# submission2019/cnn-quantization

Measured on AMD Instinct MI355X. Metric: activation elements/sec (and % HBM peak) for per-channel int4 Q/DQ, ResNet-50 b512, higher is better.
Workload: dtype f32

## Files before the change

### cnn_quantization_amd/_lib.py

```python
import ctypes
import os

from . import _build

_P = ctypes.c_void_p
_I = ctypes.c_int
_L = ctypes.c_int64
_F = ctypes.c_float

STAT_MIN, STAT_MAX, STAT_MEAN, STAT_STD, STAT_B, STAT_KURT, STAT_STD_POS, NSTAT = 0, 1, 2, 3, 4, 5, 6, 7
MOM_MIN, MOM_MAX, MOM_SUM, MOM_SUMSQ, MOM_COUNT, MOM_SUM_RELU, MOM_SUMSQ_RELU, NMOM = 0, 1, 2, 3, 4, 5, 6, 7
DEV_ABS, DEV_Z4, NDEV = 0, 1, 2
QP_SCALE, QP_ZP, QP_QMAX, NQP = 0, 1, 2, 3
MT_DELTA, MT_CMIN, MT_CMAX, MT_OMEGA, MT_ALPHA, MT_WSTART, NMT = 0, 1, 2, 3, 4, 5, 6
MT_HIST_BINS = 131072
MT_HIST_WINDOW, MT_HIST_REPLICAS = 128, 256


def mt_hist_words(C):
    return MT_HIST_BINS + 2 + 2 * C + MT_HIST_REPLICAS * MT_HIST_WINDOW + 1
KLD_BINS, KLD_QBINS, KLD_NCAND = 2001, 15, 994
DIAG_BITS, DIAG_ALPHA, DIAG_DELTA, DIAG_OFFSET, NDIAG = 0, 1, 2, 3, 4
DTYPE_F32, DTYPE_BF16, DTYPE_F16, NDTYPE = 0, 1, 2, 3

# ... 29 lines not shown
    'cnnq_pc_qdq': (_I, [_P, _P, _L, _L, _L, _P, _P, _P, _I, _P]),
    'cnnq_pc_quantize_pack4': (_I, [_P, _P, _L, _L, _L, _P, _P]),
    'cnnq_pc_dequantize_pack4': (_I, [_P, _P, _L, _L, _L, _P, _P]),
    'cnnq_pc_quantize_u8': (_I, [_P, _P, _L, _L, _L, _P, _P]),
    'cnnq_pc_dequantize_u8': (_I, [_P, _P, _L, _L, _L, _P, _P]),
    'cnnq_pc_packed_layout': (_I, [_P, _L, _L, _P, _P]),
    'cnnq_pc_quantize_packed': (_I, [_P, _P, _L, _L, _L, _P, _P, _P, _P]),
    'cnnq_pc_quantize_packed_form': (_I, [_P, _P, _L, _L, _L, _P, _P, _P, _I, _P]),
    'cnnq_pc_dequantize_packed': (_I, [_P, _P, _L, _L, _L, _P, _P, _P, _P]),
    'cnnq_pc_dequantize_packed_form': (_I, [_P, _P, _L, _L, _L, _P, _P, _P, _I, _P]),
    'cnnq_xrank_window_bytes': (ctypes.c_size_t, [_I, _I]),
    'cnnq_xrank_alloc': (_I, [_I, _I, _P, _P]),
    'cnnq_pc_minmax_qdq_xrank': (_I, [_P, _P, _L, _L, _L, _I, _I, _P, _P, ctypes.c_size_t, _P, _I, _I, _I, ctypes.c_uint32, _P, _L,
                                      _P]),
    'cnnq_pc_minmax_qdq_xrank_dev': (_I, [_P, _P, _L, _L, _L, _I, _I, _P, _P, ctypes.c_size_t, _P, _I, _I, _I, _P, _P, _L, _P, _P, _P]),
    'cnnq_pc_minmax_qdq_xrank_seq': (_I, [_P, _P, _L, _L, _L, _I, _I, _P, _P, ctypes.c_size_t, _P, _I, _I, _I, ctypes.c_uint32, _P, _I, _P, _L,
                                          _P, _P, _P]),
    'cnnq_hist_replicas_fold': (_I, [_P, _P, _P]),
    'cnnq_pc_minmax': (_I, [_P, _L, _L, _L, _P, _P]),
    'cnnq_pc_minmax_strided': (_I, [_P, _L, _L, _L, _L, _P, _P]),
    'cnnq_pc_qdq_strided': (_I, [_P, _P, _L, _L, _L, _L, _P, _P, _P, _I, _P]),
    'cnnq_pc_minmax_reduce': (_I, [_P, _I, _L, _P, _P]),
    'cnnq_pc_minmax_params': (_I, [_P, _I, _L, _I, _I, _P, _P]),
    'cnnq_pc_minmax_qdq': (_I, [_P, _P, _L, _L, _L, _I, _I, _P, _P, _P, _P, _P]),
    'cnnq_pc_resident_describe': (_I, [_L, _L, _L, ctypes.POINTER(ctypes.c_int32)]),
    'cnnq_pc_minmax_qdq_resident': (_I, [_P, _P, _L, _L, _L, _I, _I, _P, _P, _P]),
    'cnnq_group_ws_alloc': (_I, [ctypes.c_size_t, ctypes.POINTER(ctypes.c_void_p)]),
    'cnnq_group_ws_free': (_I, [_P]),
    'cnnq_group_ws_status': (_I, [_P, ctypes.POINTER(ctypes.c_uint32)]),
    'cnnq_group_ws_status_clear': (_I, [_P]),
    'cnnq_pc_group_workspace': (ctypes.c_size_t, [_L, _L, _L]),
    'cnnq_group_ws_at_rest': (_I, [_P, ctypes.POINTER(ctypes.c_uint64)]),
    'cnnq_pc_group_describe': (_I, [_L, _L, _L, ctypes.POINTER(ctypes.c_int32)]),
    'cnnq_pc_minmax_qdq_group': (_I, [_P, _P, _L, _L, _L, _I, _I, _P, _P, _P, ctypes.c_uint32, _P]),
    'cnnq_pc_minmax_local': (_I, [_P, _L, _L, _L, _P, _P, _P]),
    'cnnq_pc_minmax_local_auto': (_I, [_P, _L, _L, _L, _P, _P, ctypes.c_size_t, _P, _P]),
    'cnnq_pc_gathered_qdq': (_I, [_P, _P, _L, _L, _L, _P, _I, _I, _I, _P, _P]),
    'cnnq_pc_minmax_qdq_workspace': (ctypes.c_size_t, [_L, _L, _L]),
    'cnnq_pc_minmax_qdq_auto': (_I, [_P, _P, _L, _L, _L, _I, _I, _P, _P, ctypes.c_size_t, _I, _P]),
    'cnnq_hist_replica_bytes': (ctypes.c_size_t, []),
    'cnnq_pc_minmax_qdq_single': (_I, [_P, _P, _L, _L, _L, _I, _I, _P, ctypes.c_size_t, _P, _P, _P, _P, _P, _P]),
    'cnnq_entropy_replicas': (_I, [_P, _P, _P]),
    'cnnq_entropy_replicas_batch': (_I, [_P, _I, _P, _P]),
    'cnnq_midtread_entropy_batch': (_I, [_I, _P, _P, _P, _P, _P, _P]),
    'cnnq_pc_aciq_workspace': (ctypes.c_size_t, [_L, _L, _L, _I]),
    'cnnq_pc_aciq_qdq': (_I, [_P, _P, _L, _L, _L, ctypes.POINTER(ParamsCfg), _P, _P, _P, _P]),
    'cnnq_pc_aciq_qdq_single': (_I, [_P, _P, _L, _L, _L, ctypes.POINTER(ParamsCfg), _P, _P, ctypes.c_size_t, _P, _P, _P, _P, _P,
                                     ctypes.c_uint32, _P]),
    'cnnq_pc_aciq_qdq_auto': (_I, [_P, _P, _L, _L, _L, ctypes.POINTER(ParamsCfg), _P, _P, ctypes.c_size_t, _P, _P, _P]),
    'cnnq_pc_aciq_fused_xrank': (_I, [_P, _P, _L, _L, _L, ctypes.POINTER(ParamsCfg), _P, _P, ctypes.c_size_t, _P, _P, _P, _P,
                                      ctypes.POINTER(XRankCtx), ctypes.c_uint32, _P]),
    'cnnq_pc_midtread_fused_xrank': (_I, [_P, _P, _L, _L, _L, ctypes.c_double, _I, _P, _I, _P, _P, ctypes.c_size_t, _P, _P, _P, _P,
                                          ctypes.POINTER(XRankCtx), ctypes.c_uint32, _P]),
    'cnnq_pc_stats_xrank': (_I, [_P, _L, _L, _L, _I, _I, _I, _P, _P, ctypes.c_size_t, _P, _P, ctypes.POINTER(XRankCtx), ctypes.c_uint32,
                                 _P]),
    'cnnq_pc_weight_correct': (_I, [_P, _L, _L, _P, _P, _I, _I, _P]),
    'cnnq_pc_bcorr_sums': (_I, [_P, _P, _L, _L, _L, _I, _P, _P]),
    'cnnq_pc_qdq_bcorr_sums': (_I, [_P, _L, _L, _L, _P, _I, _P, _P]),
    'cnnq_pc_qdq_bcorr': (_I, [_P, _P, _L, _L, _L, _P, _P, _I, _P]),
    'cnnq_pc_bcorr_bias': (_I, [_P, _I, _L, _P, _P, _P]),
    'cnnq_pc_bcorr_apply': (_I, [_P, _L, _L, _L, _P, _P]),
    'cnnq_pc_midtread_params': (_I, [_P, _L, ctypes.c_double, _I, _I, _P, _I, _P, _P]),
    'cnnq_pc_midtread_qdq': (_I, [_P, _P, _L, _L, _L, _P, _I, _P, _P, _P]),
    'cnnq_pc_midtread_qdq_single': (_I, [_P, _P, _L, _L, _L, ctypes.c_double, _I, _P, _I, _P, _P, ctypes.c_size_t, _P, _P, _P,
                                         ctypes.c_uint32, _P]),
    'cnnq_midtread_entropy': (_I, [_P, _P, _L, _L, _P, _P]),
# ... 93 lines not shown
```

### cnn_quantization_amd/csrc/cnnq_group.hip.h

```cpp
#pragma once
#include "cnnq_common.hip.h"
#include "cnnq_qdq.hip.h"
#include "cnnq_xrank.hip.h"
#include "cnnq_resident.hip.h"

namespace {

constexpr long long GRP_TIMEOUT_TICKS = 2000000;
constexpr long long GRP_TIMEOUT_SHORT = 50000;
constexpr int GRP_TIMEOUT_SPINS = 1 << 20;
constexpr int GRP_CNT_STRIDE = 64;
constexpr int GRP_GS_MAX = 512;
constexpr int GRP_GS_BIG = 704;
#ifndef GRP_ACQUIRE
#define GRP_ACQUIRE 0
#endif
constexpr int GRP_SUB = 16;
#ifndef GRP_K32_WAVES
#define GRP_K32_WAVES 3
#endif

#ifdef GRP_TRACE
__device__ unsigned long long* g_grp_trace = nullptr;
#define GRP_STAMP(i)                                                                                     \
// ... 311 lines not shown
                expired = (now - t0 > timeout_ticks || spins > GRP_TIMEOUT_SPINS) ? 1 : 0;
            }
            if (__builtin_amdgcn_readfirstlane(expired)) {
                if ((tid & 63) == 0) atomicOr(sh_code, 1);
                return;
            }
            if (spins < 2) __builtin_amdgcn_s_sleep(8);
            else if (spins < 6) __builtin_amdgcn_s_sleep(32);
            else __builtin_amdgcn_s_sleep(64);
        }
    }
    if (!whole_wg) {
        for (int m = L >> 1; m >= 1; m >>= 1) { tn = pmin(tn, shfl_xor_f(tn, m)); tx = pmax(tx, shfl_xor_f(tx, m)); }
        if (active && j == 0) { sh_mn[ch] = tn; sh_mx[ch] = tx; }
    }
}

struct GWs {
    unsigned* status;
    unsigned* cnt;
    unsigned long long* part;
    unsigned long long* slots;
    int gstride;
};

#ifndef FLAT_ABL
#define FLAT_ABL 0
#endif
#if FLAT_ABL & 1
#define FLAT_ABL_NOSTORE(o) && (o)[0] == 3.0e38f
#else
#define FLAT_ABL_NOSTORE(o)
#endif
template <int A, int K, int OUT = 0, bool XR = false>
__global__ void __launch_bounds__(TPB, (K == 32 ? GRP_K32_WAVES : 1)) k_mmq_group(
    const float* __restrict__ x, float* __restrict__ y, const Geo g, const int Gs, const int num_bits, const int positive,
    const GWs ws, float* __restrict__ qp, float* __restrict__ mm, const unsigned flags, const XOut xo = XOut{},
    const XRank xr = XRank{}) {
    if constexpr (XR) xr_prologue(xr);
    __shared__ float l_mn[TPB * A], l_mx[TPB * A];
    extern __shared__ unsigned cnnq_dyn_lds[];
    unsigned* const sh_hist = cnnq_dyn_lds;
    if constexpr (OUT == 1) {
        if (xo.hist) xhist_zero(sh_hist, 1 << (num_bits < 8 ? num_bits : 8));
    }
    __shared__ float sh_mn[MAXCH], sh_mx[MAXCH], sh_sc[MAXCH], sh_zp[MAXCH], sh_rs[MAXCH];
    __shared__ int sh_timed_out, sh_slow;
    if (threadIdx.x == 0) sh_slow = 0;
    const unsigned st0 = threadIdx.x == 0 ? __hip_atomic_load(ws.status, __ATOMIC_RELAXED, __HIP_MEMORY_SCOPE_AGENT) : 0u;
    GRP_STAMP(0);
    const RBlk rb = rblk_of(g, Gs);
    const Blk& b = rb.b;
    const int tid = threadIdx.x;
    const int col = b.col0 + tid;
    const bool ok = col < b.col1;
    const int colc = ok ? col : b.col0;
    const int nrows = b.n1 - b.n0;
    const size_t base = (size_t)b.n0 * (size_t)g.P + (size_t)colc * 4;

    float v[K][4];
#pragma unroll
    for (int j = 0; j < K; ++j) {
        const int r = j < nrows ? j : nrows - 1;
        ldv_nt<4>(x + base + (size_t)r * (size_t)g.P, v[j]);
    }
    __builtin_amdgcn_sched_barrier(0);
    GRP_STAMP(1);
    float mn[A], mx[A];
    bool nan = false;
#pragma unroll
    for (int a = 0; a < A; ++a) { mn[a] = INFINITY; mx[a] = -INFINITY; }
#pragma unroll
    for (int j = 0; j < K; ++j) lane_acc<A>(v[j], mn, mx, nan);
    if (A == 1 && nan) { mn[0] = NAN; mx[0] = NAN; }
    wg_channel_minmax<A>(g, b, ok, mn, mx, l_mn, l_mx, sh_mn, sh_mx);
    const int nch = b.c1 - b.c0;
    GRP_STAMP(2);

    unsigned long long* blk = ws.part + (size_t)rb.group * ws.gstride;
    const int kk = (g.mode == 1) ? 1 : g.k;
    const bool use_slots = (flags & MMQ_FLAG_SLOTS) != 0;
    unsigned long long* slots = ws.slots + (size_t)rb.group * ws.gstride;
    if (use_slots) {
        for (int ch = tid; ch < nch; ch += TPB)
            __hip_atomic_store(slots + (size_t)rb.member * kk + ch, slot_of(sh_mn[ch], sh_mx[ch]), __ATOMIC_RELAXED,
                               __HIP_MEMORY_SCOPE_AGENT);
        if (tid == 0) sh_timed_out = ((flags & MMQ_FLAG_TEST_HOOK) ? 2 : 0) | ((st0 & 1u) ? 4 : 0);
        __syncthreads();
        GRP_STAMP(3);
    } else {
    for (int ch = tid; ch < nch; ch += TPB)
        __hip_atomic_store(blk + (size_t)rb.member * kk + ch, pack_pair(sh_mn[ch], sh_mx[ch]), __ATOMIC_RELAXED,
                           __HIP_MEMORY_SCOPE_AGENT);
    asm volatile("s_waitcnt vmcnt(0)" ::: "memory");
    __syncthreads();
    GRP_STAMP(3);
    }
    float sn = INFINITY, sx = -INFINITY;
#if FLAT_ABL & 2
    if (tid == 0) sh_timed_out = 0;
    __syncthreads();
    if (true) {
    } else
#else
    if (use_slots) {
        const int c0 = sh_timed_out;
// ... 75 lines not shown
#pragma unroll
    for (int a = 0; a < A; ++a) {
        const unsigned e = (unsigned)colc * 4u + (unsigned)a;
        const int ch = (int)(e / (unsigned)g.HW) - b.c0;
        sc[a] = sh_sc[ch];
        zp[a] = sh_zp[ch];
    }

    unsigned nzp[A];
#pragma unroll
    for (int a = 0; a < A; ++a) nzp[a] = 0u;
    if (!__builtin_amdgcn_readfirstlane(sh_slow)) {
        float rs[A];
#pragma unroll
        for (int a = 0; a < A; ++a) {
            const unsigned e = (unsigned)colc * 4u + (unsigned)a;
            rs[a] = sh_rs[(int)(e / (unsigned)g.HW) - b.c0];
        }
#pragma unroll
        for (int j = 0; j < K; ++j) {
            if (j < nrows) {
                float o[4], cd[4];
                if constexpr (A == 1) {
                    qdq4_fast(v[j], sc[0], rs[0], zp[0], qm, o, cd);
                } else {
#pragma unroll
                    for (int e = 0; e < 4; ++e) o[e] = qdq1_fast(v[j][e], sc[e], rs[e], zp[e], qm, cd[e]);
                }
                if (ok FLAT_ABL_NOSTORE(o))
                    xstore<OUT, A>(xo, reinterpret_cast<char*>(y), xo.codes, xo.packed, (base + (size_t)j * (size_t)g.P) * 4, o,
                                   cd, sh_hist, zp, nzp);
            }
        }
    } else {
#pragma unroll
        for (int j = 0; j < K; ++j) {
            if (j < nrows) {
                float o[4], cd[4];
#pragma unroll
                for (int e = 0; e < 4; ++e) o[e] = qdq1(v[j][e], sc[A == 1 ? 0 : e], zp[A == 1 ? 0 : e], qm, cd[e]);
                if (ok FLAT_ABL_NOSTORE(o))
                    xstore<OUT, A>(xo, reinterpret_cast<char*>(y), xo.codes, xo.packed, (base + (size_t)j * (size_t)g.P) * 4, o,
                                   cd, sh_hist, zp, nzp);
            }
        }
    }
    if constexpr (OUT == 1) {
        if (xo.hist) xhist_flush<A>(sh_hist, xo.hist, 1 << (num_bits < 8 ? num_bits : 8), zp, nzp);
    }
    GRP_STAMP(6);
#if !(FLAT_ABL & 2)
    if (use_slots) {
        if (tid == 0) sh_timed_out = grp_depart_last(grp_lines(ws.cnt, rb.group, Gs, 0, 1), rb.member, Gs) ? 1 : 0;
        __syncthreads();
        if (sh_timed_out)
            for (int m = tid; m < Gs * kk; m += TPB) __hip_atomic_store(slots + m, 0ull, __ATOMIC_RELAXED, __HIP_MEMORY_SCOPE_AGENT);
    } else if (tid == 0) grp_depart(grp_lines(ws.cnt, rb.group, Gs, 0, 1), rb.member, Gs);
#endif
#ifdef GRP_TRACE
    if (g_grp_trace) {
        asm volatile("s_waitcnt vmcnt(0)" ::: "memory");
        __syncthreads();
        if (tid == 0) {
            g_grp_trace[(size_t)blockIdx.x * 16 + 8] = wall_clock64();
            g_grp_trace[(size_t)blockIdx.x * 16 + 7] = ((unsigned long long)__builtin_amdgcn_s_getreg((31 << 11) | 20) << 32) |
                                                       (unsigned)__builtin_amdgcn_s_getreg((31 << 11) | 4);
        }
    }
#endif
}

struct FGeo {
    int N, C, HW, P;
    unsigned cpc;
    unsigned total;
    int Gs;
// ... 414 lines not shown
```

### cnn_quantization_amd/csrc/cnnq_kernels.hip

```cpp

#include <string.h>

#include <vector>
#include "cnnq_common.hip.h"
#include "cnnq_stats.hip.h"
#include "cnnq_params.hip.h"
#include "cnnq_qdq.hip.h"
#include "cnnq_pack4.hip.h"
#include "cnnq_midtread.hip.h"
#include "cnnq_corrections.hip.h"
#include "cnnq_pertensor.hip.h"
#include "cnnq_resident.hip.h"
#include "cnnq_group.hip.h"
#include "cnnq_plan.hip.h"
#include "cnnq_kld.hip.h"
#include "cnnq_half.hip.h"
#include "cnnq_half_stats.hip.h"
#include "cnnq_half_bcorr.hip.h"
#include "cnnq_nhwc.hip.h"
#include "cnnq_nhwc_aciq.hip.h"
#include "cnnq_nhwc_collect.hip.h"
#include "cnnq_nhwc_bcorr.hip.h"
#include "cnnq_nhwc_midtread.hip.h"
#include "cnnq_nhwc_entropy.hip.h"
// ... 563 lines not shown
int cnnq_group_ws_status(const void* ws, uint32_t* status_host) {
    if (!ws || !status_host) return CNNQ_EINVAL;
    return (int)hipMemcpy(status_host, ws, sizeof(uint32_t), hipMemcpyDeviceToHost);
}

int cnnq_group_ws_status_clear(void* ws) {
    if (!ws) return CNNQ_EINVAL;
    const uint32_t zero = 0;
    return (int)hipMemcpy(ws, &zero, sizeof(uint32_t), hipMemcpyHostToDevice);
}

int cnnq_group_ws_at_rest(const void* ws, uint64_t* nonzero_words_host) {
    if (!ws || !nonzero_words_host) return CNNQ_EINVAL;
    std::vector<uint32_t> h(GRP_WS_PAIRS / 4);
    const hipError_t e = hipMemcpy(h.data(), ws, GRP_WS_PAIRS, hipMemcpyDeviceToHost);
    if (e != hipSuccess) return (int)e;
    constexpr size_t ptf0 = PTF_OFF / 4, ptf1 = (PTF_OFF + 256 + (size_t)PTF_MAX_ROWS * 16) / 4;
    uint64_t n = 0;
    for (size_t i = 1; i < h.size(); ++i) n += (i < ptf0 || i >= ptf1) && h[i] != 0u;
    *nonzero_words_host = n;
    return 0;
}

#ifdef GRP_TRACE
int cnnq_debug_group_trace(void* buf) {
    unsigned long long* p = reinterpret_cast<unsigned long long*>(buf);
    return (int)hipMemcpyToSymbol(HIP_SYMBOL(g_grp_trace), &p, sizeof(p));
}
#endif

int cnnq_pc_group_describe(int64_t N, int64_t C, int64_t HW, int32_t out[8]) {
    if (!out) return CNNQ_EINVAL;
    GPlan p;
    const int rc = plan_group(N, C, HW, true, &p, true, 1);
    if (rc) return rc;
    const int32_t vals[8] = {p.v.A, p.K + p.KL, p.g.mode, p.g.S, p.g.ncb, p.Gs, p.ngroups, p.g.S * p.g.ncb};
    for (int i = 0; i < 8; ++i) out[i] = vals[i];
    return 0;
}

int cnnq_pc_minmax_qdq_group(const float* x, float* y, int64_t N, int64_t C, int64_t HW, int num_bits, int positive,
                             void* ws, float* qp, float* mm, unsigned flags, void* stream) {
    if (!x || !y || !ws || !qp || num_bits < 1 || num_bits > 32 || misaligned(ws, 128)) return CNNQ_EINVAL;
    GPlan p;
    const int rc = plan_group(N, C, HW, al16(x) && al16(y), &p, true, flat_lds_rows(0, false));
    if (rc) return rc;
    return launch_group(x, y, p, num_bits, positive ? 1 : 0, ws, qp, mm, flags, (hipStream_t)stream);
}

int cnnq_pc_minmax_local(const float* x, int64_t N, int64_t C, int64_t HW, float* pmm, float* local, void* stream) {
    if (!x || !pmm || !local) return CNNQ_EINVAL;
    const int G = cnnq_pc_groups(N, C, HW, al16(x) ? 1 : 0);
    if (G <= 0) return g_error(G);
    const int rc = cnnq_pc_minmax(x, N, C, HW, pmm, stream);
    if (rc) return rc;
    return cnnq_pc_minmax_reduce(pmm, G, C, local, stream);
}

int cnnq_pc_minmax_local_auto(const float* x, int64_t N, int64_t C, int64_t HW, float* pmm, void* gws, size_t gws_bytes,
                              float* local, void* stream) {
    if (!x || !local) return CNNQ_EINVAL;
    static const int64_t max_bytes = env_int("CNNQ_LOCAL_GROUP_MAX_MB", 384) * ((int64_t)1 << 20);
    if (gws && !misaligned(gws, 128) && N * C * HW * 4 <= max_bytes) {
        GPlan p;
        if (plan_group(N, C, HW, al16(x), &p, false) == 0 && p.ws_bytes <= gws_bytes)
            return launch_minmax_group(x, p, gws, local, (hipStream_t)stream);
    }
    return cnnq_pc_minmax_local(x, N, C, HW, pmm, local, stream);
}

int cnnq_pc_gathered_qdq(const float* x, float* y, int64_t N, int64_t C, int64_t HW, const float* gathered, int W,
                         int num_bits, int positive, float* qp, void* stream) {
    if (!x || !y || !gathered || W <= 0 || num_bits < 1 || num_bits > 32) return CNNQ_EINVAL;
    Variant v;
    Geo g;
    const int rc = plan(N, C, HW, al16(x) && al16(y), 1, &v, &g, 1);
    if (rc) return rc;
    const GathArgs ga{W, num_bits, positive ? 1 : 0, qp};
// ... 20 lines not shown
}

int cnnq_pc_minmax_qdq_auto(const float* x, float* y, int64_t N, int64_t C, int64_t HW, int num_bits, int positive,
                            float* ws, void* gws, size_t gws_bytes, int allow_single_launch, void* stream) {
    if (!x || !y || !ws || num_bits < 1 || num_bits > 32 || C <= 0) return CNNQ_EINVAL;
    const MmWs w(ws, C);
    if (allow_single_launch) {
        const size_t gneed = gws ? cnnq_pc_group_workspace(N, C, HW) : 0;
        WPlan wp;
        int route = mm_route(N, C, HW, al16(x) && al16(y), gneed > 0 && gneed <= gws_bytes, &wp);
        if (route == ROUTE_GROUP) {
            const int rc = cnnq_pc_minmax_qdq_group(x, y, N, C, HW, num_bits, positive, gws, w.qp, w.mm, 0u, stream);
            if (rc != CNNQ_ENOTSUP) return rc;
            route = mm_route(N, C, HW, al16(x) && al16(y), false, &wp);
        }
        if (route == ROUTE_WHOLE) return launch_whole(x, y, wp, num_bits, positive ? 1 : 0, w.qp, w.mm, hs(stream));
    }
    return cnnq_pc_minmax_qdq(x, y, N, C, HW, num_bits, positive, w.pmm, w.qp, nullptr, nullptr, stream);
}

size_t cnnq_hist_replica_bytes(void) { return (size_t)XHIST_REPLICAS * 256 * sizeof(unsigned long long); }

int cnnq_pc_minmax_qdq_single(const float* x, float* y, int64_t N, int64_t C, int64_t HW, int num_bits, int positive,
                              void* gws, size_t gws_bytes, float* qp, float* mm, uint8_t* codes, uint64_t* hist_rep,
                              uint8_t* packed, void* stream) {
    if (!x || !qp || num_bits < 1 || num_bits > 32 || C <= 0) return CNNQ_EINVAL;
    if (packed ? (y || codes || hist_rep || num_bits > 4 || misaligned(packed, 2)) : !y) return CNNQ_EINVAL;
    if ((codes || hist_rep) && num_bits > 8) return CNNQ_EINVAL;
    if (misaligned(codes, 4) || misaligned(hist_rep, 8) || misaligned(gws, 128)) return CNNQ_EINVAL;
    const int out = packed ? 2 : (codes || hist_rep) ? 1 : 0;
    const XOut xo = xout(codes, hist_rep, packed);
    const bool al = al16(x) && (packed ? true : al16(y));
    GPlan gp;
    const bool group_ok = gws && plan_group(N, C, HW, al, &gp, true, flat_lds_rows(out, false)) == 0 && gp.ws_bytes <= gws_bytes;
    WPlan wp;
    switch (mm_route(N, C, HW, al, group_ok, &wp)) {
    case ROUTE_WHOLE: return launch_whole(x, y, wp, num_bits, positive ? 1 : 0, qp, mm, hs(stream), out, xo);
    case ROUTE_GROUP: return launch_group(x, y, gp, num_bits, positive ? 1 : 0, gws, qp, mm, 0u, hs(stream), out, xo);
    }
    return CNNQ_ENOTSUP;
}

size_t cnnq_xrank_window_bytes(int world, int cmax) {
    return (world > 0 && cmax > 0) ? xr_window_bytes(world, cmax) : 0;
}

int cnnq_xrank_alloc(int world, int cmax, void** window, unsigned char handle[64]) {
    if (!window || !handle || world <= 0 || cmax <= 0) return CNNQ_EINVAL;
    const size_t bytes = xr_window_bytes(world, cmax);
    hipError_t e = hipExtMallocWithFlags(window, bytes, hipDeviceMallocUncached);
    if (e != hipSuccess) return (int)e;
    e = hipMemset(*window, 0, bytes);
    hipIpcMemHandle_t h;
    if (e == hipSuccess) e = hipIpcGetMemHandle(&h, *window);
    if (e == hipSuccess) e = hipDeviceSynchronize();
    if (e != hipSuccess) {
        (void)hipFree(*window);
        *window = nullptr;
        return (int)e;
    }
    memcpy(handle, &h, 64);
    return 0;
}

static int xrank_launch(const float* x, float* y, int64_t N, int64_t C, int64_t HW, int num_bits, int positive, float* ws, void* gws,
                        size_t gws_bytes, void* const* windows, int rank, int world, int cmax, uint32_t seq, uint32_t* seq_dev,
                        uint32_t* status, int64_t timeout_ticks, uint8_t* codes, uint64_t* hist_rep, void* stream, int zero_c = 0,
// ... 1377 lines not shown
```

### cnn_quantization_amd/csrc/cnnq_plan.hip.h

```cpp
#pragma once
#include <stdio.h>
#include "cnnq_common.hip.h"
#include "cnnq_resident.hip.h"
#include "cnnq_group.hip.h"
#include "cnnq_aciq.hip.h"
#include "cnnq_stats1.hip.h"

namespace {

int gcd_i(int a, int b) { return b ? gcd_i(b, a % b) : a; }

constexpr int MAXG = 64;

int choose_variant(int64_t N, int64_t C, int64_t HW, bool aligned16, Variant* v) {
    if (aligned16 && HW % 4 == 0) {
        const int64_t cpc = HW / 4;
        int J = 4;
        if (cpc <= TPB * 4) {
            const int64_t smax = N < MAXG ? N : MAXG;
            for (J = 4; J > 1; J >>= 1) {
                const int64_t cap = TPB * J;
                const int64_t ncb = (cpc > cap) ? C * ((cpc + cap - 1) / cap) : (C + cap / cpc - 1) / (cap / cpc);
                static const int64_t minwgs = env_int("CNNQ_PLAN_MINWGS", 2048);
                if (ncb * smax >= minwgs) break;
// ... 278 lines not shown
    int64_t Gs = (total + TPB * (K + KL) - 1) / (TPB * (K + KL));
    int64_t gs_max = grp_gs_max();
    if (Gs > gs_max && K == 32 && lds_rows >= 1) {
        KL = 8;
        Gs = (total + TPB * (K + KL) - 1) / (TPB * (K + KL));
        gs_max = grp_gs_big();
    }
    if (Gs > gs_max || Gs < 2) return CNNQ_ENOTSUP;
    const int64_t rows = (TPB * (K + KL)) / cpc + 3;
    if (rows * C * HW * 4 >= (int64_t)1 << 32) return CNNQ_ENOTSUP;
    const int64_t nsub = (Gs + GRP_SUB - 1) / GRP_SUB;
    if (C * (nsub > 1 ? nsub + 1 : 1) > GRP_MAX_LINES) return CNNQ_ENOTSUP;
    p->flat = 1;
    p->KL = KL;
    p->v = {4, 1, 1};
    p->K = K;
    p->Gs = (int)Gs;
    p->ngroups = (int)C;
    p->gstride = (int)(((Gs + 15) / 16) * 16);
    p->ws_bytes = GRP_WS_PAIRS + (size_t)C * p->gstride * 8;
    FGeo& f = p->fg;
    f.N = (int)N; f.C = (int)C; f.HW = (int)HW; f.P = (int)(C * HW);
    f.cpc = (unsigned)cpc; f.total = (unsigned)total; f.Gs = (int)Gs;
    f.q256 = (unsigned)(TPB / cpc); f.r16 = (unsigned)(TPB % cpc) * 16u; f.rs = (unsigned)(C * HW * 4);
    static const int cb_knob = env_int("CNNQ_GRP_CB", 4);
    const int64_t cb_fit = ((int64_t)chip_cus() * 3 / 2) / Gs;
    f.cb = (int)(cb_knob > 1 ? (cb_fit < cb_knob ? (cb_fit < 1 ? 1 : cb_fit) : cb_knob) : 1);
    p->g = Geo{};
    p->g.N = (int)N; p->g.C = (int)C; p->g.HW = (int)HW; p->g.P = (int)(C * HW);
    p->g.mode = 3; p->g.S = (int)Gs; p->g.ncb = (int)C; p->g.Cn = (int)C; p->g.nb = 1; p->g.k = 1;
    return 0;
}

int plan_group_compute(int64_t N, int64_t C, int64_t HW, bool aligned16, GPlan* p, bool allow_flat, int lds_rows, int a4_kmax);

inline int flat_lds_rows(int out, bool xrank) {
    static const int kl_knob = env_int("CNNQ_FLAT_KL", 0);
    return (out == 1 || xrank) ? 0 : (kl_knob == 8 ? 2 : 1);
}

int plan_group(int64_t N, int64_t C, int64_t HW, bool aligned16, GPlan* p, bool allow_flat = true, int lds_rows = 0, int a4_kmax = 32) {
    struct Entry { int64_t N, C, HW; int key, rc; GPlan plan; };
    constexpr int SLOTS = 64;
    thread_local Entry cache[SLOTS];
    thread_local int used = 0, next = 0;
    const int key = (aligned16 ? 1 : 0) | (allow_flat ? 2 : 0) | (lds_rows << 2) | (a4_kmax << 4);
    for (int i = 0; i < used; ++i)
        if (cache[i].N == N && cache[i].C == C && cache[i].HW == HW && cache[i].key == key) {
            *p = cache[i].plan;
            return cache[i].rc;
        }
    const int rc = plan_group_compute(N, C, HW, aligned16, p, allow_flat, lds_rows, a4_kmax);
    Entry& e = cache[next];
    e.N = N; e.C = C; e.HW = HW; e.key = key; e.rc = rc; e.plan = *p;
    next = (next + 1) % SLOTS;
    if (used < SLOTS) ++used;
    return rc;
}

int plan_rows(int64_t N, int64_t C, int64_t HW, GPlan* p, int a4_kmax = 32);
inline int plan_sums(int64_t N, int64_t C, int64_t HW, bool aligned16, GPlan* p, int lds_rows) {
    return plan_group(N, C, HW, aligned16, p, true, lds_rows, 16);
}

int plan_group_compute(int64_t N, int64_t C, int64_t HW, bool aligned16, GPlan* p, bool allow_flat, int lds_rows, int a4_kmax) {
    if (N <= 0 || C <= 0 || HW <= 0) return CNNQ_EINVAL;
    if (!aligned16) return CNNQ_ENOTSUP;
    p->flat = 0;
    p->KL = 0;
    if (allow_flat && plan_flat(N, C, HW, p, lds_rows, false) == 0) return 0;
    const int rc = plan_rows(N, C, HW, p, a4_kmax);
    if (rc != CNNQ_ENOTSUP || !allow_flat || lds_rows == 0) return rc;
    GPlan q;
    if (plan_flat(N, C, HW, &q, lds_rows, true) != 0 || q.KL != 8) return rc;
    *p = q;
    return 0;
}

int plan_rows(int64_t N, int64_t C, int64_t HW, GPlan* p, int a4_kmax) {
    p->flat = 0;
    p->KL = 0;
    if (HW % 4 == 0) {
        p->v = {4, 1, 1};
    } else if ((C * HW) % 4 == 0) {
        const int m = 4 / gcd_i((int)(HW % 4), 4);
        if ((int64_t)m * HW > TPB * 4) return CNNQ_ENOTSUP;
        p->v = {4, 4, 1};
    } else {
        return CNNQ_ENOTSUP;
    }
    const int rc = make_geo(N, C, HW, p->v, 0, C, 0, 0, 0, &p->g);
    if (rc) return rc;
    Geo& g = p->g;
    static const int forceK = env_int("CNNQ_GRP_K", 0);
    static const int target = env_int("CNNQ_GRP_WGS", 1024);
    const int members_per_split = (g.mode == 1) ? g.nb : 1;
    int K = 4;
    if (forceK == 4 || forceK == 8 || forceK == 16 || forceK == 32) {
        K = forceK;
    } else {
        for (K = 32; K > 4; K >>= 1)
            if ((int64_t)g.ncb * ((N + K - 1) / K) >= target) break;
    }
    if (p->v.A == 4 && K > a4_kmax) K = a4_kmax;
    const int kcap = p->v.A == 4 ? a4_kmax : 32;
    while (K < kcap && ((N + K - 1) / K) * members_per_split > grp_gs_max()) K <<= 1;
    const int64_t S = (N + K - 1) / K;
    if (S * members_per_split > grp_gs_max()) return CNNQ_ENOTSUP;
    if (S * g.ncb >= (int64_t)1 << 31) return CNNQ_ERANGE;
    g.S = (int)S;
    p->K = K;
    p->Gs = (int)(S * members_per_split);
    p->ngroups = (g.mode == 1) ? g.Cn : g.ncb;
    {
        const int64_t nsub = (p->Gs + GRP_SUB - 1) / GRP_SUB;
        if ((int64_t)p->ngroups * (nsub > 1 ? nsub + 1 : 1) > GRP_MAX_LINES) return CNNQ_ENOTSUP;
    }
    const int64_t pairs = (int64_t)p->Gs * ((g.mode == 1) ? 1 : g.k);
    p->gstride = (int)(((pairs + 15) / 16) * 16);
    p->ws_bytes = GRP_WS_PAIRS + (size_t)p->ngroups * p->gstride * 8;
    return 0;
}

inline bool slots_fit(const GPlan& p, int words = 1) { return (size_t)p.ngroups * p.gstride * words * 8 <= GRP_WS_SLOT_BYTES; }

int launch_group(const float* x, float* y, const GPlan& p, int num_bits, int positive, void* ws, float* qp, float* mm,
                 unsigned flags, hipStream_t st, int out = 0, const XOut& xo = XOut{}, const XRank* xrp = nullptr) {
    flags |= mmq_env_flags();
    const bool xrank = xrp && xrp->world > 0;
    if (xrank && out == 2) return CNNQ_ENOTSUP;
    const XRank xr = xrank ? *xrp : XRank{};
    const size_t hb = xhist_lds_bytes(out, xo.hist, 1 << (num_bits < 8 ? num_bits : 8));
    const GWs w = gws_view(ws, p.gstride);
    const dim3 grid((unsigned)((int64_t)p.g.S * p.g.ncb)), block(TPB);
    if (!(flags & MMQ_FLAG_COUNTERS) && slots_fit(p)) flags |= MMQ_FLAG_SLOTS;
    if (p.flat) {
        const dim3 fgrid((unsigned)((int64_t)p.fg.C * p.fg.Gs));
        static const int pk_narrow = env_int("CNNQ_PK_NARROW", 0);
        if (out == 2 && (pk_narrow || ((uintptr_t)xo.packed & 15))) flags |= MMQ_FLAG_PK_NARROW;
        static const int pk_plain = env_int("CNNQ_PK_PLAIN", 0);
        if (out == 2 && pk_plain) flags |= MMQ_FLAG_PK_PLAIN;
        FGeo fg = p.fg;
        static const int cb_forced = env_int("CNNQ_GRP_CB", 0);
        if (out == 2 && !cb_forced) fg.cb = 1;
        const bool lds = p.K == 32 && p.KL == 8;
        if (lds && (xrank || out == 1)) return CNNQ_EINVAL;
        with_int<32, 16, 8>(p.K, [&](auto k) {
            with_int<0, 1, 2>(out, [&](auto o) {
                with_bool(xrank, lds, [&](auto xc, auto l) {
                    constexpr int K = decltype(k)::value, OUT = decltype(o)::value, KL = decltype(l)::value ? 8 : 0;
                    constexpr bool XR = decltype(xc)::value;
                    if constexpr (!(XR && OUT == 2) && !(KL && (K != 32 || XR || OUT == 1)))
                        hipLaunchKernelGGL((k_mmq_flat<K, OUT, XR, KL>), fgrid, block, hb, st, x, y, fg, num_bits, positive, w, qp, mm, flags, xo, xr);
                });
            });
        });
        return launch_status();
    }
    with_int<4, 1>(p.v.A, [&](auto a) {
        with_int<32, 16, 8, 4>(p.K, [&](auto k) {
            with_int<0, 1, 2>(out, [&](auto o) {
                with_bool(xrank, [&](auto xc) {
                    constexpr int A = decltype(a)::value, K = decltype(k)::value, OUT = decltype(o)::value;
                    constexpr bool XR = decltype(xc)::value;
                    if constexpr (!(XR && OUT == 2))
                        hipLaunchKernelGGL((k_mmq_group<A, K, OUT, XR>), grid, block, hb, st, x, y, p.g, p.Gs, num_bits, positive, w, qp, mm, flags, xo, xr);
                });
            });
        });
    });
    return launch_status();
}

inline bool fused_ok(int mode, const GPlan& p, int out) {
    if (!slots_fit(p)) return false;
    if (p.KL && !(p.flat && p.K == 32 && p.KL == 8)) return false;
    if (mode == 1 && !p.flat && p.v.A != 1) return false;
    if (mode == 0 && !p.flat && p.v.A == 4 && p.K == 32) return false;
    if (p.KL && mode == 0 && out == 1) return false;
    return true;
}
inline bool plan_fused(int mode, int64_t N, int64_t C, int64_t HW, bool aligned16, size_t gws_bytes, int out, GPlan* p) {
    return plan_sums(N, C, HW, aligned16, p, (mode == 0 && out == 1) ? 0 : 1) == 0 && p->ws_bytes <= gws_bytes && fused_ok(mode, *p, out);
}

int launch_fused(int mode, const float* x, float* y, const GPlan& p, const FusedArgs& fa, void* ws, unsigned flags, hipStream_t st,
                 int out, const XOut& xo, const XRank* xrp = nullptr) {
    const bool xrank = xrp && xrp->world > 0;
    if (xrank && mode == 0 && out == 1) return CNNQ_ENOTSUP;
    const XRank xr = xrank ? *xrp : XRank{};
    if (!fused_ok(mode, p, out)) return CNNQ_ENOTSUP;
// ... 111 lines not shown
```

### cnn_quantization_amd/csrc/cnnq_qdq.hip.h

```cpp
#pragma once
#include "cnnq_common.hip.h"
#include "cnnq_params.hip.h"

namespace {

__device__ __forceinline__ float qdq1(float x, float scale, float zp, float qmax, float& code) {
    float q = x / scale;
    q = q + zp;
    q = (q > qmax) ? qmax : q;
    q = (q < 0.f) ? 0.f : q;
    q = rintf(q);
    code = q;
    return (q - zp) * scale;
}

constexpr unsigned MMQ_FLAG_TEST_HOOK = 1u;
constexpr unsigned MMQ_FLAG_IEEE_DIVIDE = 2u;
constexpr unsigned MMQ_FLAG_SLOTS = 16u;
constexpr unsigned MMQ_FLAG_COUNTERS = 32u;
constexpr unsigned MMQ_FLAG_PK_PLAIN = 8u;
constexpr unsigned MMQ_FLAG_PK_NARROW = 4u;

__device__ __forceinline__ bool qdq_fast_domain(float cmn, float cmx, float scale) {
    return fabsf(cmn) <= 0x1p70f && fabsf(cmx) <= 0x1p70f && scale <= 0x1p30f;
}

__device__ __forceinline__ float qdq1_fast(float x, float scale, float rs, float zp, float qmax, float& code) {
    float q = x * rs;
    float r = __builtin_fmaf(-scale, q, x);
    q = __builtin_fmaf(r, rs, q);
    r = __builtin_fmaf(-scale, q, x);
    q = __builtin_fmaf(r, rs, q);
    q = q + zp;
    q = __builtin_amdgcn_fmed3f(q, 0.f, qmax);
    q = rintf(q);
    code = q;
    return (q - zp) * scale;
}

typedef float f2v __attribute__((ext_vector_type(2)));
__device__ __forceinline__ f2v qdq2_fast(f2v x, f2v s, f2v rs, f2v zp, float qmax, f2v& code) {
    f2v q = x * rs;
    f2v r = __builtin_elementwise_fma(-s, q, x);
    q = __builtin_elementwise_fma(r, rs, q);
    r = __builtin_elementwise_fma(-s, q, x);
    q = __builtin_elementwise_fma(r, rs, q);
    q = q + zp;
    q.x = rintf(__builtin_amdgcn_fmed3f(q.x, 0.f, qmax));
    q.y = rintf(__builtin_amdgcn_fmed3f(q.y, 0.f, qmax));
    code = q;
    return (q - zp) * s;
}
// ... 444 lines not shown
```

### include/cnnq_hip.h

```cpp
#ifndef CNNQ_HIP_H
#define CNNQ_HIP_H

#include <stddef.h>
#include <stdint.h>

#ifdef __cplusplus
extern "C" {
#endif

#define CNNQ_EINVAL (-1)
#define CNNQ_ERANGE (-2)
#define CNNQ_ENOTSUP (-3)

enum {
    CNNQ_STAT_MIN = 0,
    CNNQ_STAT_MAX = 1,
    CNNQ_STAT_MEAN = 2,
    CNNQ_STAT_STD = 3,
    CNNQ_STAT_B = 4,
    CNNQ_STAT_KURT = 5,
    CNNQ_STAT_STD_POS = 6,
    CNNQ_NSTAT = 7
};

// ... 81 lines not shown
                          void* stream);

int cnnq_pc_packed_layout(const float* bits, int64_t C, int64_t HW, uint32_t* rowoff, void* stream);
int cnnq_pc_quantize_packed(const float* x, uint8_t* packed, int64_t N, int64_t C, int64_t HW, const float* qp,
                            const float* bits, const uint32_t* rowoff, void* stream);
int cnnq_pc_quantize_packed_form(const float* x, uint8_t* packed, int64_t N, int64_t C, int64_t HW, const float* qp,
                                 const float* bits, const uint32_t* rowoff, int form, void* stream);
int cnnq_pc_dequantize_packed_form(const uint8_t* packed, float* y, int64_t N, int64_t C, int64_t HW, const float* qp,
                                   const float* bits, const uint32_t* rowoff, int form, void* stream);
int cnnq_pc_dequantize_packed(const uint8_t* packed, float* y, int64_t N, int64_t C, int64_t HW, const float* qp,
                              const float* bits, const uint32_t* rowoff, void* stream);

int cnnq_pc_minmax(const float* x, int64_t N, int64_t C, int64_t HW, float* pmm, void* stream);
int cnnq_pc_minmax_strided(const float* x, int64_t N, int64_t C, int64_t HW, int64_t sample_stride, float* pmm,
                           void* stream);
int cnnq_pc_qdq_strided(const float* x, float* y, int64_t N, int64_t C, int64_t HW, int64_t sample_stride,
                        const float* qp, uint8_t* codes, uint64_t* hist, int reverse, void* stream);
int cnnq_pc_minmax_reduce(const float* pmm, int G, int64_t C, float* out, void* stream);
int cnnq_pc_minmax_params(const float* pmm, int G, int64_t C, int num_bits, int positive, float* qp, void* stream);
int cnnq_pc_minmax_qdq(const float* x, float* y, int64_t N, int64_t C, int64_t HW, int num_bits, int positive,
                       float* pmm, float* qp, uint8_t* codes, uint64_t* hist, void* stream);

int cnnq_pc_resident_describe(int64_t N, int64_t C, int64_t HW, int32_t out[8]);
int cnnq_pc_minmax_qdq_resident(const float* x, float* y, int64_t N, int64_t C, int64_t HW, int num_bits, int positive,
                                float* qp, float* mm, void* stream);

size_t cnnq_pc_group_workspace(int64_t N, int64_t C, int64_t HW);
int cnnq_group_ws_alloc(size_t bytes, void** ws);
int cnnq_group_ws_free(void* ws);
int cnnq_group_ws_status(const void* ws, uint32_t* status_host);
int cnnq_group_ws_status_clear(void* ws);
int cnnq_group_ws_at_rest(const void* ws, uint64_t* nonzero_words_host);
int cnnq_pc_group_describe(int64_t N, int64_t C, int64_t HW, int32_t out[8]);
int cnnq_pc_minmax_qdq_group(const float* x, float* y, int64_t N, int64_t C, int64_t HW, int num_bits, int positive,
                             void* ws, float* qp, float* mm, unsigned flags, void* stream);

int cnnq_pc_minmax_local(const float* x, int64_t N, int64_t C, int64_t HW, float* pmm, float* local, void* stream);
int cnnq_pc_minmax_local_auto(const float* x, int64_t N, int64_t C, int64_t HW, float* pmm, void* gws, size_t gws_bytes,
                              float* local, void* stream);
int cnnq_pc_gathered_qdq(const float* x, float* y, int64_t N, int64_t C, int64_t HW, const float* gathered, int W,
                         int num_bits, int positive, float* qp, void* stream);

size_t cnnq_pc_minmax_qdq_workspace(int64_t N, int64_t C, int64_t HW);
int cnnq_pc_minmax_qdq_auto(const float* x, float* y, int64_t N, int64_t C, int64_t HW, int num_bits, int positive,
                            float* ws, void* gws, size_t gws_bytes, int allow_single_launch, void* stream);

size_t cnnq_hist_replica_bytes(void);
int cnnq_pc_minmax_qdq_single(const float* x, float* y, int64_t N, int64_t C, int64_t HW, int num_bits, int positive,
                              void* gws, size_t gws_bytes, float* qp, float* mm, uint8_t* codes, uint64_t* hist_rep,
                              uint8_t* packed, void* stream);
int cnnq_entropy_replicas(uint64_t* hist_rep, float* out, void* stream);
int cnnq_entropy_replicas_batch(uint64_t* hist_rep, int n, float* out, void* stream);

size_t cnnq_xrank_window_bytes(int world, int cmax);
int cnnq_xrank_alloc(int world, int cmax, void** window, unsigned char handle[64]);
int cnnq_xrank_open(const unsigned char handle[64], void** window);
int cnnq_xrank_close(void* window);
int cnnq_xrank_free(void* window);
int cnnq_pc_minmax_qdq_xrank(const float* x, float* y, int64_t N, int64_t C, int64_t HW, int num_bits, int positive,
                             float* ws, void* gws, size_t gws_bytes, void* const* windows, int rank, int world, int cmax,
                             uint32_t seq, uint32_t* status, int64_t timeout_ticks, void* stream);
int cnnq_pc_minmax_qdq_xrank_dev(const float* x, float* y, int64_t N, int64_t C, int64_t HW, int num_bits, int positive,
                                 float* ws, void* gws, size_t gws_bytes, void* const* windows, int rank, int world, int cmax,
                                 uint32_t* seq_dev, uint32_t* status, int64_t timeout_ticks, uint8_t* codes, uint64_t* hist_rep,
                                 void* stream);
int cnnq_pc_minmax_qdq_xrank_seq(const float* x, float* y, int64_t N, int64_t C, int64_t HW, int num_bits, int positive,
// ... 155 lines not shown
```

Measured before the change: 647.2 billion.

## Stage extra rows per group workgroup through LDS via direct-to-LDS loads

```diff
diff --git a/cnn_quantization_amd/_lib.py b/cnn_quantization_amd/_lib.py
--- a/cnn_quantization_amd/_lib.py
+++ b/cnn_quantization_amd/_lib.py
@@ -85,6 +85,7 @@
     'cnnq_pc_group_workspace': (ctypes.c_size_t, [_L, _L, _L]),
     'cnnq_group_ws_at_rest': (_I, [_P, ctypes.POINTER(ctypes.c_uint64)]),
     'cnnq_pc_group_describe': (_I, [_L, _L, _L, ctypes.POINTER(ctypes.c_int32)]),
+    'cnnq_pc_group_describe_flags': (_I, [_L, _L, _L, ctypes.c_uint32, ctypes.POINTER(ctypes.c_int32)]),
     'cnnq_pc_minmax_qdq_group': (_I, [_P, _P, _L, _L, _L, _I, _I, _P, _P, _P, ctypes.c_uint32, _P]),
     'cnnq_pc_minmax_local': (_I, [_P, _L, _L, _L, _P, _P, _P]),
     'cnnq_pc_minmax_local_auto': (_I, [_P, _L, _L, _L, _P, _P, ctypes.c_size_t, _P, _P]),
diff --git a/cnn_quantization_amd/csrc/cnnq_group.hip.h b/cnn_quantization_amd/csrc/cnnq_group.hip.h
--- a/cnn_quantization_amd/csrc/cnnq_group.hip.h
+++ b/cnn_quantization_amd/csrc/cnnq_group.hip.h
@@ -367,7 +367,7 @@
 #else
 #define FLAT_ABL_NOSTORE(o)
 #endif
-template <int A, int K, int OUT = 0, bool XR = false>
+template <int A, int K, int OUT = 0, bool XR = false, int KL = 0>
 __global__ void __launch_bounds__(TPB, (K == 32 ? GRP_K32_WAVES : 1)) k_mmq_group(
     const float* __restrict__ x, float* __restrict__ y, const Geo g, const int Gs, const int num_bits, const int positive,
     const GWs ws, float* __restrict__ qp, float* __restrict__ mm, const unsigned flags, const XOut xo = XOut{},
@@ -381,6 +381,7 @@
     }
     __shared__ float sh_mn[MAXCH], sh_mx[MAXCH], sh_sc[MAXCH], sh_zp[MAXCH], sh_rs[MAXCH];
     __shared__ int sh_timed_out, sh_slow;
+    __shared__ __attribute__((aligned(16))) float sh_x[KL ? KL * TPB * 4 : 4];
     if (threadIdx.x == 0) sh_slow = 0;
     const unsigned st0 = threadIdx.x == 0 ? __hip_atomic_load(ws.status, __ATOMIC_RELAXED, __HIP_MEMORY_SCOPE_AGENT) : 0u;
     GRP_STAMP(0);
@@ -399,6 +400,14 @@
         const int r = j < nrows ? j : nrows - 1;
         ldv_nt<4>(x + base + (size_t)r * (size_t)g.P, v[j]);
     }
+    if constexpr (KL > 0) {
+        const char* xt = reinterpret_cast<const char*>(x + (size_t)b.n0 * (size_t)g.P);
+#pragma unroll
+        for (int l = 0; l < KL; ++l) {
+            const int r = K + l < nrows ? K + l : nrows - 1;
+            lds_dma16_behind(xt, ((unsigned)r * (unsigned)g.P + (unsigned)colc * 4u) * 4u, sh_x + (l * TPB + (threadIdx.x & ~63)) * 4);
+        }
+    }
     __builtin_amdgcn_sched_barrier(0);
     GRP_STAMP(1);
     float mn[A], mx[A];
@@ -407,6 +416,15 @@
     for (int a = 0; a < A; ++a) { mn[a] = INFINITY; mx[a] = -INFINITY; }
 #pragma unroll
     for (int j = 0; j < K; ++j) lane_acc<A>(v[j], mn, mx, nan);
+    if constexpr (KL > 0) {
+        lds_dma_landed(mn[0]);
+#pragma unroll
+        for (int l = 0; l < KL; ++l) {
+            const float4 q = *reinterpret_cast<const float4*>(sh_x + (l * TPB + tid) * 4);
+            const float t[4] = {q.x, q.y, q.z, q.w};
+            lane_acc<A>(t, mn, mx, nan);
+        }
+    }
     if (A == 1 && nan) { mn[0] = NAN; mx[0] = NAN; }
     wg_channel_minmax<A>(g, b, ok, mn, mx, l_mn, l_mx, sh_mn, sh_mx);
     const int nch = b.c1 - b.c0;
@@ -548,6 +566,25 @@
                                    cd, sh_hist, zp, nzp);
             }
         }
+        if constexpr (KL > 0) {
+#pragma unroll
+            for (int l = 0; l < KL; ++l) {
+                if (K + l < nrows) {
+                    const float4 q = *reinterpret_cast<const float4*>(sh_x + (l * TPB + tid) * 4);
+                    const float t[4] = {q.x, q.y, q.z, q.w};
+                    float o[4], cd[4];
+                    if constexpr (A == 1) {
+                        qdq4_fast(t, sc[0], rs[0], zp[0], qm, o, cd);
+                    } else {
+#pragma unroll
+                        for (int e = 0; e < 4; ++e) o[e] = qdq1_fast(t[e], sc[e], rs[e], zp[e], qm, cd[e]);
+                    }
+                    if (ok)
+                        xstore<OUT, A>(xo, reinterpret_cast<char*>(y), xo.codes, xo.packed, (base + (size_t)(K + l) * (size_t)g.P) * 4, o,
+                                       cd, sh_hist, zp, nzp);
+                }
+            }
+        }
     } else {
 #pragma unroll
         for (int j = 0; j < K; ++j) {
@@ -558,6 +595,21 @@
                 if (ok FLAT_ABL_NOSTORE(o))
                     xstore<OUT, A>(xo, reinterpret_cast<char*>(y), xo.codes, xo.packed, (base + (size_t)j * (size_t)g.P) * 4, o,
                                    cd, sh_hist, zp, nzp);
+            }
+        }
+        if constexpr (KL > 0) {
+#pragma unroll
+            for (int l = 0; l < KL; ++l) {
+                if (K + l < nrows) {
+                    const float4 q = *reinterpret_cast<const float4*>(sh_x + (l * TPB + tid) * 4);
+                    const float t[4] = {q.x, q.y, q.z, q.w};
+                    float o[4], cd[4];
+#pragma unroll
+                    for (int e = 0; e < 4; ++e) o[e] = qdq1(t[e], sc[A == 1 ? 0 : e], zp[A == 1 ? 0 : e], qm, cd[e]);
+                    if (ok)
+                        xstore<OUT, A>(xo, reinterpret_cast<char*>(y), xo.codes, xo.packed, (base + (size_t)(K + l) * (size_t)g.P) * 4, o,
+                                       cd, sh_hist, zp, nzp);
+                }
             }
         }
     }
diff --git a/cnn_quantization_amd/csrc/cnnq_kernels.hip b/cnn_quantization_amd/csrc/cnnq_kernels.hip
--- a/cnn_quantization_amd/csrc/cnnq_kernels.hip
+++ b/cnn_quantization_amd/csrc/cnnq_kernels.hip
@@ -619,9 +619,20 @@
 int cnnq_pc_group_describe(int64_t N, int64_t C, int64_t HW, int32_t out[8]) {
     if (!out) return CNNQ_EINVAL;
     GPlan p;
-    const int rc = plan_group(N, C, HW, true, &p, true, 1);
+    const int rc = plan_group(N, C, HW, true, &p, true, 1, 32, grp_rows_kl(0, false));
     if (rc) return rc;
     const int32_t vals[8] = {p.v.A, p.K + p.KL, p.g.mode, p.g.S, p.g.ncb, p.Gs, p.ngroups, p.g.S * p.g.ncb};
+    for (int i = 0; i < 8; ++i) out[i] = vals[i];
+    return 0;
+}
+
+int cnnq_pc_group_describe_flags(int64_t N, int64_t C, int64_t HW, unsigned flags, int32_t out[8]) {
+    if (!out) return CNNQ_EINVAL;
+    GPlan p;
+    const int rc = (flags & 256u) ? plan_sums(N, C, HW, true, &p, 1)
+                                  : plan_group(N, C, HW, true, &p, true, flat_lds_rows(0, false), 32, grp_rows_kl(0, false, flags));
+    if (rc) return rc;
+    const int32_t vals[8] = {p.v.A, p.K, p.KL, p.g.mode, p.g.S, p.Gs, p.g.S * p.g.ncb, (int32_t)((p.ws_bytes + 1023) >> 10)};
     for (int i = 0; i < 8; ++i) out[i] = vals[i];
     return 0;
 }
@@ -630,7 +641,7 @@
                              void* ws, float* qp, float* mm, unsigned flags, void* stream) {
     if (!x || !y || !ws || !qp || num_bits < 1 || num_bits > 32 || misaligned(ws, 128)) return CNNQ_EINVAL;
     GPlan p;
-    const int rc = plan_group(N, C, HW, al16(x) && al16(y), &p, true, flat_lds_rows(0, false));
+    const int rc = plan_group(N, C, HW, al16(x) && al16(y), &p, true, flat_lds_rows(0, false), 32, grp_rows_kl(0, false, flags));
     if (rc) return rc;
     return launch_group(x, y, p, num_bits, positive ? 1 : 0, ws, qp, mm, flags, (hipStream_t)stream);
 }
@@ -717,7 +728,7 @@
     const XOut xo = xout(codes, hist_rep, packed);
     const bool al = al16(x) && (packed ? true : al16(y));
     GPlan gp;
-    const bool group_ok = gws && plan_group(N, C, HW, al, &gp, true, flat_lds_rows(out, false)) == 0 && gp.ws_bytes <= gws_bytes;
+    const bool group_ok = gws && plan_group(N, C, HW, al, &gp, true, flat_lds_rows(out, false), 32, grp_rows_kl(out, false)) == 0 && gp.ws_bytes <= gws_bytes;
     WPlan wp;
     switch (mm_route(N, C, HW, al, group_ok, &wp)) {
     case ROUTE_WHOLE: return launch_whole(x, y, wp, num_bits, positive ? 1 : 0, qp, mm, hs(stream), out, xo);
diff --git a/cnn_quantization_amd/csrc/cnnq_plan.hip.h b/cnn_quantization_amd/csrc/cnnq_plan.hip.h
--- a/cnn_quantization_amd/csrc/cnnq_plan.hip.h
+++ b/cnn_quantization_amd/csrc/cnnq_plan.hip.h
@@ -334,25 +334,32 @@
     return 0;
 }
 
-int plan_group_compute(int64_t N, int64_t C, int64_t HW, bool aligned16, GPlan* p, bool allow_flat, int lds_rows, int a4_kmax);
+int plan_group_compute(int64_t N, int64_t C, int64_t HW, bool aligned16, GPlan* p, bool allow_flat, int lds_rows, int a4_kmax, int rows_kl);
 
 inline int flat_lds_rows(int out, bool xrank) {
     static const int kl_knob = env_int("CNNQ_FLAT_KL", 0);
     return (out == 1 || xrank) ? 0 : (kl_knob == 8 ? 2 : 1);
 }
-
-int plan_group(int64_t N, int64_t C, int64_t HW, bool aligned16, GPlan* p, bool allow_flat = true, int lds_rows = 0, int a4_kmax = 32) {
+inline int grp_rows_kl(int out, bool xrank, unsigned flags = 0u) {
+    static const int kl_knob = env_int("CNNQ_GRP_KL", -1);
+    if (out != 0 || xrank) return 0;
+    if (flags & MMQ_FLAG_LDS_ROWS) return 2;
+    return kl_knob == 0 ? 0 : kl_knob == 8 ? 2 : 1;
+}
+
+int plan_group(int64_t N, int64_t C, int64_t HW, bool aligned16, GPlan* p, bool allow_flat = true, int lds_rows = 0, int a4_kmax = 32,
+               int rows_kl = 0) {
     struct Entry { int64_t N, C, HW; int key, rc; GPlan plan; };
     constexpr int SLOTS = 64;
     thread_local Entry cache[SLOTS];
     thread_local int used = 0, next = 0;
-    const int key = (aligned16 ? 1 : 0) | (allow_flat ? 2 : 0) | (lds_rows << 2) | (a4_kmax << 4);
+    const int key = (aligned16 ? 1 : 0) | (allow_flat ? 2 : 0) | (lds_rows << 2) | (a4_kmax << 4) | (rows_kl << 12);
     for (int i = 0; i < used; ++i)
         if (cache[i].N == N && cache[i].C == C && cache[i].HW == HW && cache[i].key == key) {
             *p = cache[i].plan;
             return cache[i].rc;
         }
-    const int rc = plan_group_compute(N, C, HW, aligned16, p, allow_flat, lds_rows, a4_kmax);
+    const int rc = plan_group_compute(N, C, HW, aligned16, p, allow_flat, lds_rows, a4_kmax, rows_kl);
     Entry& e = cache[next];
     e.N = N; e.C = C; e.HW = HW; e.key = key; e.rc = rc; e.plan = *p;
     next = (next + 1) % SLOTS;
@@ -360,18 +367,18 @@
     return rc;
 }
 
-int plan_rows(int64_t N, int64_t C, int64_t HW, GPlan* p, int a4_kmax = 32);
+int plan_rows(int64_t N, int64_t C, int64_t HW, GPlan* p, int a4_kmax = 32, int lds_rows = 0);
 inline int plan_sums(int64_t N, int64_t C, int64_t HW, bool aligned16, GPlan* p, int lds_rows) {
     return plan_group(N, C, HW, aligned16, p, true, lds_rows, 16);
 }
 
-int plan_group_compute(int64_t N, int64_t C, int64_t HW, bool aligned16, GPlan* p, bool allow_flat, int lds_rows, int a4_kmax) {
+int plan_group_compute(int64_t N, int64_t C, int64_t HW, bool aligned16, GPlan* p, bool allow_flat, int lds_rows, int a4_kmax, int rows_kl) {
     if (N <= 0 || C <= 0 || HW <= 0) return CNNQ_EINVAL;
     if (!aligned16) return CNNQ_ENOTSUP;
     p->flat = 0;
     p->KL = 0;
     if (allow_flat && plan_flat(N, C, HW, p, lds_rows, false) == 0) return 0;
-    const int rc = plan_rows(N, C, HW, p, a4_kmax);
+    const int rc = plan_rows(N, C, HW, p, a4_kmax, rows_kl);
     if (rc != CNNQ_ENOTSUP || !allow_flat || lds_rows == 0) return rc;
     GPlan q;
     if (plan_flat(N, C, HW, &q, lds_rows, true) != 0 || q.KL != 8) return rc;
@@ -379,7 +386,15 @@
     return 0;
 }
 
-int plan_rows(int64_t N, int64_t C, int64_t HW, GPlan* p, int a4_kmax) {
+inline int rows_wgs_per_cu(int K) { return K >= 32 ? GRP_K32_WAVES : K == 16 ? 5 : 8; }
+constexpr int GRP_ROWS_KL = 8;
+
+inline bool rows_kl_pays(int A, int64_t wgs, int K, int64_t wgs_kl) {
+    const int64_t slots = (int64_t)chip_cus() * rows_wgs_per_cu(K), slots_kl = (int64_t)chip_cus() * rows_wgs_per_cu(32);
+    return A == 1 && wgs > slots && wgs_kl <= slots_kl && wgs_kl >= 2 * (int64_t)chip_cus();
+}
+
+int plan_rows(int64_t N, int64_t C, int64_t HW, GPlan* p, int a4_kmax, int lds_rows) {
     p->flat = 0;
     p->KL = 0;
     if (HW % 4 == 0) {
@@ -407,11 +422,20 @@
     if (p->v.A == 4 && K > a4_kmax) K = a4_kmax;
     const int kcap = p->v.A == 4 ? a4_kmax : 32;
     while (K < kcap && ((N + K - 1) / K) * members_per_split > grp_gs_max()) K <<= 1;
-    const int64_t S = (N + K - 1) / K;
+    int KL = 0;
+    if (lds_rows && kcap == 32 && forceK == 0 && (int64_t)g.P * 4 * (32 + GRP_ROWS_KL) < ((int64_t)1 << 32)) {
+        const int64_t S_kl = (N + 32 + GRP_ROWS_KL - 1) / (32 + GRP_ROWS_KL);
+        if (lds_rows == 2 || rows_kl_pays(p->v.A, (int64_t)g.ncb * ((N + K - 1) / K), K, (int64_t)g.ncb * S_kl)) {
+            K = 32;
+            KL = GRP_ROWS_KL;
+        }
+    }
+    const int64_t S = (N + K + KL - 1) / (K + KL);
     if (S * members_per_split > grp_gs_max()) return CNNQ_ENOTSUP;
     if (S * g.ncb >= (int64_t)1 << 31) return CNNQ_ERANGE;
     g.S = (int)S;
     p->K = K;
+    p->KL = KL;
     p->Gs = (int)(S * members_per_split);
     p->ngroups = (g.mode == 1) ? g.Cn : g.ncb;
     {
@@ -459,6 +483,14 @@
         });
         return launch_status();
     }
+    if (p.KL) {
+        if (p.K != 32 || p.KL != GRP_ROWS_KL || out != 0 || xrank) return CNNQ_EINVAL;
+        with_int<4, 1>(p.v.A, [&](auto a) {
+            hipLaunchKernelGGL((k_mmq_group<decltype(a)::value, 32, 0, false, GRP_ROWS_KL>), grid, block, hb, st, x, y, p.g, p.Gs, num_bits, positive, w, qp,
+                               mm, flags, xo, xr);
+        });
+        return launch_status();
+    }
     with_int<4, 1>(p.v.A, [&](auto a) {
         with_int<32, 16, 8, 4>(p.K, [&](auto k) {
             with_int<0, 1, 2>(out, [&](auto o) {
diff --git a/cnn_quantization_amd/csrc/cnnq_qdq.hip.h b/cnn_quantization_amd/csrc/cnnq_qdq.hip.h
--- a/cnn_quantization_amd/csrc/cnnq_qdq.hip.h
+++ b/cnn_quantization_amd/csrc/cnnq_qdq.hip.h
@@ -18,6 +18,7 @@
 constexpr unsigned MMQ_FLAG_IEEE_DIVIDE = 2u;
 constexpr unsigned MMQ_FLAG_SLOTS = 16u;
 constexpr unsigned MMQ_FLAG_COUNTERS = 32u;
+constexpr unsigned MMQ_FLAG_LDS_ROWS = 64u;
 constexpr unsigned MMQ_FLAG_PK_PLAIN = 8u;
 constexpr unsigned MMQ_FLAG_PK_NARROW = 4u;
 
diff --git a/include/cnnq_hip.h b/include/cnnq_hip.h
--- a/include/cnnq_hip.h
+++ b/include/cnnq_hip.h
@@ -137,6 +137,7 @@
 int cnnq_group_ws_status_clear(void* ws);
 int cnnq_group_ws_at_rest(const void* ws, uint64_t* nonzero_words_host);
 int cnnq_pc_group_describe(int64_t N, int64_t C, int64_t HW, int32_t out[8]);
+int cnnq_pc_group_describe_flags(int64_t N, int64_t C, int64_t HW, unsigned flags, int32_t out[8]);
 int cnnq_pc_minmax_qdq_group(const float* x, float* y, int64_t N, int64_t C, int64_t HW, int num_bits, int positive,
                              void* ws, float* qp, float* mm, unsigned flags, void* stream);
 
```

Result: no change. 648.9 billion (median of 2 runs) (+0.2%).
